# hrz2000/CustomNeRF

Hardware: AMD Instinct MI355X
Metric: training rays/s (higher is better)
Workload: dtype f16

## Files before the change

### customnerf_amd/csrc/grid_fwd_eval.h

```cpp
#pragma once
#include "grid_common.h"

__device__ __forceinline__ float gf_mix_lo(float w, uint32_t g2, float negzero) {
    float r;
    asm("v_fma_mix_f32 %0, %1, %2, %3 op_sel_hi:[0,1,0]" : "=v"(r) : "v"(w), "v"(g2), "v"(negzero));
    return r;
}
__device__ __forceinline__ float gf_mix_hi(float w, uint32_t g2, float negzero) {
    float r;
    asm("v_fma_mix_f32 %0, %1, %2, %3 op_sel:[0,1,0] op_sel_hi:[0,1,0]" : "=v"(r) : "v"(w), "v"(g2), "v"(negzero));
    return r;
}
__device__ __forceinline__ void gf_accum(cn_gf_h2 &acc, float w, uint32_t g2, float negzero) {
    const float p0 = gf_mix_lo(w, g2, negzero), p1 = gf_mix_hi(w, g2, negzero);
    const cn_gf_h2 p = {(_Float16)p0, (_Float16)p1};
    acc = acc + p;
}
__device__ __forceinline__ uint32_t gf_ld1(const unsigned char *__restrict__ base, uint32_t byte_off) { return *reinterpret_cast<const uint32_t *>(base + byte_off); }
struct __attribute__((packed, aligned(4))) gf_u2 { uint32_t x, y; };
struct alignas(16) gf_u4 { uint32_t x, y, z, w; };

__device__ __forceinline__ uint32_t gf_eval_level(const float (&in)[3], const unsigned char *__restrict__ table, uint32_t size, uint32_t resolution,
                                                  float scale, uint32_t gridtype) {
    float fr[3], om[3];
    uint32_t pg[3];
#pragma unroll
    for (int d = 0; d < 3; d++) {
        const float pos = cn_fma(in[d], scale, 0.5f);
        pg[d] = (uint32_t)floorf(pos);
        fr[d] = pos - (float)pg[d];
        om[d] = 1 - fr[d];
    }
    const float a00 = om[0] * om[1], a10 = fr[0] * om[1], a01 = om[0] * fr[1], a11 = fr[0] * fr[1];
    const float w[8] = {a00 * om[2], a10 * om[2], a01 * om[2], a11 * om[2], a00 * fr[2], a10 * fr[2], a01 * fr[2], a11 * fr[2]};
    uint32_t c[8];
    const int mode = ge_level_mode<3>(gridtype, false, size, resolution);
    if (mode == GE_MODE_DENSE) {
        const uint32_t s1 = resolution + 1, s2 = s1 * s1;
        const uint32_t i00 = (pg[0] + pg[1] * s1 + pg[2] * s2) * 4u;
        const gf_u2 r0 = *reinterpret_cast<const gf_u2 *>(table + i00);
        const gf_u2 r1 = *reinterpret_cast<const gf_u2 *>(table + (i00 + s1 * 4u));
        const gf_u2 r2 = *reinterpret_cast<const gf_u2 *>(table + (i00 + s2 * 4u));
        const gf_u2 r3 = *reinterpret_cast<const gf_u2 *>(table + (i00 + (s1 + s2) * 4u));
        c[0] = r0.x; c[1] = r0.y; c[2] = r1.x; c[3] = r1.y; c[4] = r2.x; c[5] = r2.y; c[6] = r3.x; c[7] = r3.y;
    } else if (mode == GE_MODE_HASH2) {
        const uint32_t mask = size - 1;
        const uint32_t hy0 = pg[1] * 2654435761u, hy1 = hy0 + 2654435761u, hz0 = pg[2] * 805459861u, hz1 = hz0 + 805459861u;
        const uint32_t x0 = pg[0], xm = x0 ^ (x0 + 1);
        const bool in_quad = (xm & mask) < 4u;
        const bool odd = (x0 & 1u) != 0;
        const uint32_t hyz[4] = {hy0 ^ hz0, hy1 ^ hz0, hy0 ^ hz1, hy1 ^ hz1};
        uint32_t i0[4];
        gf_u4 v[4];
#pragma unroll
        for (int q = 0; q < 4; q++) {
            i0[q] = (x0 ^ hyz[q]) & mask;
            v[q] = *reinterpret_cast<const gf_u4 *>(table + ((i0[q] & ~3u) * 4u));
        }
        uint32_t far[4] = {0u, 0u, 0u, 0u};
        if (!in_quad) {
#pragma unroll
            for (int q = 0; q < 4; q++) far[q] = gf_ld1(table, ((i0[q] ^ xm) & mask) * 4u);
        }
#pragma unroll
        for (int q = 0; q < 4; q++) {
            const bool b0 = (i0[q] & 1u) != 0, b1 = (i0[q] & 2u) != 0;
            const uint32_t plo = b1 ? v[q].z : v[q].x, phi = b1 ? v[q].w : v[q].y;
            c[2 * q] = b0 ? phi : plo;
            const uint32_t same = b0 ? plo : phi;
            const uint32_t olo = b1 ? v[q].x : v[q].z, ohi = b1 ? v[q].y : v[q].w;
            const uint32_t cross = b0 ? olo : ohi;
            const uint32_t near = odd ? cross : same;
            c[2 * q + 1] = in_quad ? near : far[q];
        }
    } else {
        const uint32_t mask = size - 1, step = resolution + 1;
        const uint32_t s1 = step <= size ? step : 0u;
        const uint32_t s2 = (s1 && step * step <= size) ? step * step : 0u;
        const uint32_t lin = pg[0] + pg[1] * s1 + pg[2] * s2;
        const uint32_t row[4] = {lin, lin + s1, lin + s2, lin + s1 + s2};
        gf_u2 r[4];
        uint32_t i0[4];
#pragma unroll
        for (int q = 0; q < 4; q++) {
            i0[q] = row[q] & mask;
            r[q] = *reinterpret_cast<const gf_u2 *>(table + (i0[q] == mask ? i0[q] - 1 : i0[q]) * 4u);
        }
        bool any_wrap = false;
#pragma unroll
        for (int q = 0; q < 4; q++) any_wrap = any_wrap || i0[q] == mask;
        uint32_t first = 0u;
        if (any_wrap) first = gf_ld1(table, 0u);
#pragma unroll
        for (int q = 0; q < 4; q++) {
            const bool wrap = i0[q] == mask;
            c[2 * q] = wrap ? r[q].y : r[q].x;
            c[2 * q + 1] = wrap ? first : r[q].y;
        }
    }
    const float negzero = -0.0f;
    cn_gf_h2 acc = {(_Float16)0, (_Float16)0};
#pragma unroll
    for (int k = 0; k < 8; k++) gf_accum(acc, w[k], c[k], negzero);
    return __builtin_bit_cast(uint32_t, acc);
}
```

### customnerf_amd/csrc/gridencoder.hip

```cpp
#include "grid_common.h"

template <typename T, int D, int C>
__global__ void __launch_bounds__(GE_BLOCK) k_grid_fwd(const float *__restrict__ inputs, const T *__restrict__ grid, const GridLevels lv,
                                                       T *__restrict__ outputs, uint32_t B, uint32_t L, uint32_t n_levels, uint32_t nb,
                                                       T *__restrict__ dy_dx, uint32_t gridtype, int align_corners, uint32_t interp, int swizzle,
                                                       uint32_t ostride) {
    uint32_t level, pb;
    if (!ge_work_item(nb, n_levels, swizzle, lv, level, pb)) return;
    const uint32_t b = pb * GE_BLOCK + threadIdx.x;
    if (b >= B) return;

    using Vec = FeatVec<T, C>;
    const Vec *__restrict__ table = reinterpret_cast<const Vec *>(grid) + lv.offset[level];
    Vec *out = reinterpret_cast<Vec *>(outputs) + ((size_t)level * ostride + b);

    float in[D];
    bool oob = false;
    ge_load_coords<D>(inputs, b, in);
#pragma unroll
    for (int d = 0; d < D; d++) oob = oob || (in[d] < 0 || in[d] > 1);
    if (oob) {
        Vec z;
#pragma unroll
        for (int c = 0; c < C; c++) z.v[c] = ge_from_float<T>(0.0f);
        *out = z;
        if (dy_dx) {
            T *dd = dy_dx + (size_t)b * D * L * C + (size_t)level * D * C;
#pragma unroll
            for (int i = 0; i < D * C; i++) dd[i] = ge_from_float<T>(0.0f);
        }
        return;
    }

    const uint32_t hashmap_size = lv.size[level];
    const float scale = lv.scale[level];
    const uint32_t resolution = lv.resolution[level];

    float pos[D], pos_deriv[D];
    uint32_t pos_grid[D];
#pragma unroll
    for (int d = 0; d < D; d++) {
        pos[d] = cn_fma(in[d], scale, align_corners ? 0.0f : 0.5f);
        const float fl = floorf(pos[d]);
        pos_grid[d] = (uint32_t)fl;
        pos[d] -= (float)pos_grid[d];
        if (interp == 1) {
            pos_deriv[d] = ge_smoothstep_derivative(pos[d]);
            pos[d] = ge_smoothstep(pos[d]);
        } else {
            pos_deriv[d] = 1.0f;
        }
    }

    struct alignas(sizeof(T) * C) VecPair { Vec a, b; };
    struct alignas(sizeof(T) * C * 4) VecQuad { Vec e[4]; };
    Vec corner[1 << D];
    float wgt[1 << D];
    bool quad = false;
    if constexpr (sizeof(Vec) == 4) {
        quad = gridtype == 0 && ((lv.offset[level] | hashmap_size) & 3u) == 0 && ge_is_hashed<D>(align_corners, hashmap_size, resolution);
    }
    ge_dispatch_mode(ge_level_mode<D>(gridtype, align_corners, hashmap_size, resolution), [&](auto mode_c) {
#pragma unroll
    for (int q = 0; q < (1 << (D - 1)); q++) {
        uint32_t pgl[D];
#pragma unroll
        for (int d = 1; d < D; d++) pgl[d] = (((2 * q) & (1 << d)) == 0) ? pos_grid[d] : pos_grid[d] + 1;
        float w0 = 1 - pos[0], w1 = pos[0];
#pragma unroll
        for (int d = 1; d < D; d++) {
            const float f = (((2 * q) & (1 << d)) == 0) ? (1 - pos[d]) : pos[d];
            w0 *= f; w1 *= f;
        }
        wgt[2 * q] = w0; wgt[2 * q + 1] = w1;
        pgl[0] = pos_grid[0];
        const uint32_t i0 = ge_index_m<D, decltype(mode_c)::value>(gridtype, align_corners, hashmap_size, resolution, pgl);
        pgl[0] = pos_grid[0] + 1;
        const uint32_t i1 = ge_index_m<D, decltype(mode_c)::value>(gridtype, align_corners, hashmap_size, resolution, pgl);
        if (quad) {
            if constexpr (sizeof(Vec) == 4) {
                const VecQuad v = *reinterpret_cast<const VecQuad *>(table + (i0 & ~3u));
                const uint32_t k0 = i0 & 3u, k1 = i1 & 3u;
                const Vec a01 = (k0 & 1) ? v.e[1] : v.e[0], a23 = (k0 & 1) ? v.e[3] : v.e[2];
                corner[2 * q] = (k0 & 2) ? a23 : a01;
                const Vec b01 = (k1 & 1) ? v.e[1] : v.e[0], b23 = (k1 & 1) ? v.e[3] : v.e[2];
                Vec e1 = (k1 & 2) ? b23 : b01;
                if ((i0 ^ i1) > 3u) e1 = table[i1];
                corner[2 * q + 1] = e1;
            }
        } else {
            const uint32_t lo = min(i0, i1), hi_ = max(i0, i1);
            const uint32_t b = (lo + 1 < hashmap_size) ? lo : lo - 1;
            const VecPair v = *reinterpret_cast<const VecPair *>(table + b);
            const Vec e_lo = (b == lo) ? v.a : v.b;
            Vec e_hi = v.b;
            if (hi_ - lo != 1) e_hi = table[hi_];
            corner[2 * q] = (i0 == lo) ? e_lo : e_hi;
            corner[2 * q + 1] = (i0 == lo) ? e_hi : e_lo;
        }
    }
    });
    Vec res;
    if constexpr (sizeof(T) == 2 && C == 2) {
        __half2 r2 = __floats2half2_rn(0.0f, 0.0f);
#pragma unroll
        for (int idx = 0; idx < (1 << D); idx++) ge_accum2(r2, wgt[idx], *reinterpret_cast<const __half2 *>(&corner[idx]));
        res = *reinterpret_cast<const Vec *>(&r2);
    } else {
#pragma unroll
        for (int c = 0; c < C; c++) res.v[c] = ge_from_float<T>(0.0f);
#pragma unroll
        for (int idx = 0; idx < (1 << D); idx++) {
#pragma unroll
            for (int c = 0; c < C; c++) ge_accum(res.v[c], wgt[idx], corner[idx].v[c]);
        }
    }
    *out = res;

    if (dy_dx) {
        T *dd = dy_dx + (size_t)b * D * L * C + (size_t)level * D * C;
#pragma unroll
        for (int gd = 0; gd < D; gd++) {
            T rg[C];
#pragma unroll
            for (int c = 0; c < C; c++) rg[c] = ge_from_float<T>(0.0f);
#pragma unroll
            for (int idx = 0; idx < (1 << (D - 1)); idx++) {
                float w = scale;
                uint32_t pgl[D];
#pragma unroll
                for (int nd = 0; nd < D - 1; nd++) {
                    const int d = (nd >= gd) ? (nd + 1) : nd;
                    if ((idx & (1 << nd)) == 0) { w *= 1 - pos[d]; pgl[d] = pos_grid[d]; }
                    else { w *= pos[d]; pgl[d] = pos_grid[d] + 1; }
                }
                pgl[gd] = pos_grid[gd];
                const Vec left = table[ge_index<D>(gridtype, align_corners, hashmap_size, resolution, pgl)];
                pgl[gd] = pos_grid[gd] + 1;
                const Vec right = table[ge_index<D>(gridtype, align_corners, hashmap_size, resolution, pgl)];
#pragma unroll
                for (int c = 0; c < C; c++) {
                    if constexpr (sizeof(T) == 2) {
                        const float diff = __half2float(__float2half_rn(ge_opaque(__half2float(right.v[c]) - __half2float(left.v[c]))));
                        const float prod = ge_opaque(w * diff * pos_deriv[gd]);
                        rg[c] = __float2half_rn(ge_opaque(__half2float(rg[c]) + __half2float(__float2half_rn(prod))));
                    } else {
                        const float diff = right.v[c] - left.v[c];
                        rg[c] = cn_fma(w * diff, pos_deriv[gd], rg[c]);
                    }
                }
            }
#pragma unroll
            for (int c = 0; c < C; c++) dd[gd * C + c] = rg[c];
        }
    }
}

#include "grid_fwd_eval.h"

__global__ void __launch_bounds__(GE_BLOCK) k_grid_fwd_fast(const float *__restrict__ inputs, const __half *__restrict__ grid, const GridLevels lv,
                                                            __half *__restrict__ outputs, uint32_t B, uint32_t n_levels, uint32_t nb, uint32_t gridtype,
                                                            int swizzle, uint32_t ostride) {
    uint32_t level, pb;
    if (!ge_work_item(nb, n_levels, swizzle, lv, level, pb)) return;
    const uint32_t b = pb * GE_BLOCK + threadIdx.x;
    if (b >= B) return;
    uint32_t *out = reinterpret_cast<uint32_t *>(outputs) + ((size_t)level * ostride + b);
    float in[3];
    ge_load_coords<3>(inputs, b, in);
    if (in[0] < 0 || in[0] > 1 || in[1] < 0 || in[1] > 1 || in[2] < 0 || in[2] > 1) { *out = 0u; return; }

    const unsigned char *__restrict__ table = reinterpret_cast<const unsigned char *>(grid) + (size_t)lv.offset[level] * 4;
    *out = gf_eval_level(in, table, lv.size[level], lv.resolution[level], lv.scale[level], gridtype);
}

template <int SPT>
__global__ void __launch_bounds__(GE_BLOCK) k_grid_fwd_fast_sm(const float *__restrict__ inputs, const __half *__restrict__ grid, const GridLevels lv,
                                                               __half *__restrict__ outputs, uint32_t B, uint32_t n_levels, uint32_t gridtype,
                                                               uint32_t ostride) {
    const uint32_t t0 = blockIdx.x * (GE_BLOCK * SPT) + threadIdx.x;
    if (t0 >= B) return;
    float in[SPT][3];
    bool ok[SPT];
#pragma unroll
    for (int s = 0; s < SPT; s++) {
        ge_load_coords<3>(inputs, min(t0 + s * GE_BLOCK, B - 1), in[s]);
        ok[s] = !(in[s][0] < 0 || in[s][0] > 1 || in[s][1] < 0 || in[s][1] > 1 || in[s][2] < 0 || in[s][2] > 1);
#pragma unroll
        for (int d = 0; d < 3; d++) in[s][d] = ok[s] ? in[s][d] : 0.5f;
    }
    uint32_t *out = reinterpret_cast<uint32_t *>(outputs);
    for (uint32_t i = 0; i < n_levels; i++) {
        const uint32_t level = lv.order[i];
        const unsigned char *__restrict__ table = reinterpret_cast<const unsigned char *>(grid) + (size_t)lv.offset[level] * 4;
        const uint32_t size = lv.size[level], res = lv.resolution[level];
        const float scale = lv.scale[level];
#pragma unroll
        for (int s = 0; s < SPT; s++) {
            const uint32_t b = t0 + s * GE_BLOCK;
            const uint32_t r = gf_eval_level(in[s], table, size, res, scale, gridtype);
            if (b < B) out[(size_t)level * ostride + b] = ok[s] ? r : 0u;
        }
    }
}

template <typename T, int D, int C>
__global__ void __launch_bounds__(GE_BLOCK) k_grid_bwd(const T *__restrict__ grad, const float *__restrict__ inputs, const GridLevels lv,
                                                       float *__restrict__ grad_grid, uint32_t B, uint32_t n_levels, uint32_t nb,
                                                       uint32_t gridtype, int align_corners, uint32_t interp, int swizzle, float *__restrict__ found_inf) {
    uint32_t level, pb;
    if (!ge_work_item(nb, n_levels, swizzle, lv, level, pb)) return;
    const uint32_t b = pb * GE_BLOCK + threadIdx.x;
    if (b >= B) return;

    float in[D];
#pragma unroll
    for (int d = 0; d < D; d++) {
        in[d] = inputs[(size_t)b * D + d];
        if (in[d] < 0 || in[d] > 1) return;
    }
    using Vec = FeatVec<T, C>;
    const Vec g = reinterpret_cast<const Vec *>(grad)[(size_t)level * B + b];
    float *__restrict__ gtable = grad_grid + (size_t)lv.offset[level] * C;
    const uint32_t hashmap_size = lv.size[level];
    const float scale = lv.scale[level];
    const uint32_t resolution = lv.resolution[level];

    float pos[D];
    uint32_t pos_grid[D];
#pragma unroll
    for (int d = 0; d < D; d++) {
        pos[d] = cn_fma(in[d], scale, align_corners ? 0.0f : 0.5f);
        pos_grid[d] = (uint32_t)floorf(pos[d]);
        pos[d] -= (float)pos_grid[d];
        if (interp == 1) pos[d] = ge_smoothstep(pos[d]);
    }
    float gf[C];
#pragma unroll
    for (int c = 0; c < C; c++) {
        gf[c] = ge_to_float(g.v[c]);
        if (!(fabsf(gf[c]) <= 3.4e38f) && found_inf) *found_inf = 1.0f;
    }
#pragma unroll
    for (int idx = 0; idx < (1 << D); idx++) {
        float w = 1;
        uint32_t pgl[D];
#pragma unroll
        for (int d = 0; d < D; d++) {
            if ((idx & (1 << d)) == 0) { w *= 1 - pos[d]; pgl[d] = pos_grid[d]; }
            else { w *= pos[d]; pgl[d] = pos_grid[d] + 1; }
        }
        const uint32_t index = ge_index<D>(gridtype, align_corners, hashmap_size, resolution, pgl) * C;
#pragma unroll
        for (int c = 0; c < C; c++) unsafeAtomicAdd(&gtable[index + c], w * gf[c]);
    }
}

template <typename T, int D, int C>
__global__ void __launch_bounds__(GE_BLOCK) k_input_bwd(const T *__restrict__ grad, const T *__restrict__ dy_dx, float *__restrict__ grad_inputs,
                                                        uint32_t B, uint32_t L) {
    const uint32_t t = threadIdx.x + blockIdx.x * blockDim.x;
    if (t >= B * D) return;
    const uint32_t b = t / D, d = t - b * D;
    const T *dd = dy_dx + (size_t)b * L * D * C;
    float result = 0;
    for (uint32_t l = 0; l < L; l++) {
#pragma unroll
        for (int c = 0; c < C; c++)
            result = cn_fma(ge_to_float(grad[(size_t)l * B * C + (size_t)b * C + c]), ge_to_float(dd[l * D * C + d * C + c]), result);
    }
    grad_inputs[t] = result;
}

template <int D, int C>
__global__ void __launch_bounds__(GE_BLOCK) k_grad_tv(const float *__restrict__ inputs, const float *__restrict__ grid, float *__restrict__ grad,
                                                      const GridLevels lv, float weight, uint32_t B, uint32_t n_levels, uint32_t nb,
                                                      uint32_t gridtype, int align_corners) {
    uint32_t level, pb;
    if (!ge_work_item(nb, n_levels, 0, lv, level, pb)) return;
    const uint32_t b = pb * GE_BLOCK + threadIdx.x;
    if (b >= B) return;
    float in[D];
#pragma unroll
    for (int d = 0; d < D; d++) {
        in[d] = inputs[(size_t)b * D + d];
        if (in[d] < 0 || in[d] > 1) return;
    }
    const float *__restrict__ table = grid + (size_t)lv.offset[level] * C;
    float *__restrict__ gtable = grad + (size_t)lv.offset[level] * C;
    const uint32_t hashmap_size = lv.size[level], resolution = lv.resolution[level];
    const float scale = lv.scale[level];
    uint32_t pos_grid[D];
#pragma unroll
    for (int d = 0; d < D; d++) pos_grid[d] = (uint32_t)floorf(cn_fma(in[d], scale, align_corners ? 0.0f : 0.5f));
    float results[C], idelta[C];
#pragma unroll
    for (int c = 0; c < C; c++) { results[c] = 0; idelta[c] = 0; }
    const uint32_t index = ge_index<D>(gridtype, align_corners, hashmap_size, resolution, pos_grid) * C;
    const float w = weight / (2 * D);
#pragma unroll
    for (int d = 0; d < D; d++) {
        const uint32_t cur_d = pos_grid[d];
        if (cur_d < resolution) {
            pos_grid[d] = cur_d + 1;
            const uint32_t ir = ge_index<D>(gridtype, align_corners, hashmap_size, resolution, pos_grid) * C;
#pragma unroll
            for (int c = 0; c < C; c++) {
                const float gv = table[index + c] - table[ir + c];
                results[c] += gv;
                idelta[c] = cn_fma(gv, gv, idelta[c]);
            }
        }
        if (cur_d > 0) {
            pos_grid[d] = cur_d - 1;
            const uint32_t il = ge_index<D>(gridtype, align_corners, hashmap_size, resolution, pos_grid) * C;
#pragma unroll
            for (int c = 0; c < C; c++) {
                const float gv = table[index + c] - table[il + c];
                results[c] += gv;
                idelta[c] = cn_fma(gv, gv, idelta[c]);
            }
        }
        pos_grid[d] = cur_d;
    }
#pragma unroll
    for (int c = 0; c < C; c++) unsafeAtomicAdd(&gtable[index + c], w * results[c] * (1.0f / sqrtf(idelta[c] + 1e-9f)));
}

__global__ void __launch_bounds__(256) k_cast_f32_f16(const float *__restrict__ src, __half *__restrict__ dst, uint64_t n) {
    const uint64_t n8 = n / 8;
    const uint64_t stride = (uint64_t)gridDim.x * blockDim.x;
    for (uint64_t i = (uint64_t)blockIdx.x * blockDim.x + threadIdx.x; i < n8; i += stride) {
        const float4 a = reinterpret_cast<const float4 *>(src)[i * 2], b = reinterpret_cast<const float4 *>(src)[i * 2 + 1];
        union { __half2 h[4]; uint4 u; } o;
        o.h[0] = __floats2half2_rn(a.x, a.y);
        o.h[1] = __floats2half2_rn(a.z, a.w);
        o.h[2] = __floats2half2_rn(b.x, b.y);
        o.h[3] = __floats2half2_rn(b.z, b.w);
        reinterpret_cast<uint4 *>(dst)[i] = o.u;
    }
    for (uint64_t i = n8 * 8 + (uint64_t)blockIdx.x * blockDim.x + threadIdx.x; i < n; i += stride) dst[i] = __float2half_rn(src[i]);
}

static int ge_swizzle_default() {
    static const int v = cn_tune_env("CNERF_GRID_SWIZZLE", 2);
    return v;
}
static double ge_dense_weight() {
    static const double w = cn_tune_env_f("CNERF_GRID_DENSE_W", 0.7);
    return w;
}

static bool ge_fast_eligible(const GridLevels &lv, uint32_t nl, uint32_t gridtype) {
    static const int on = cn_tune_env("CNERF_GRID_FAST", 1);
    if (!on) return false;
    for (uint32_t l = 0; l < nl; l++) {
        const uint64_t step = (uint64_t)lv.resolution[l] + 1, cells = step * step * step;
        const uint32_t size = lv.size[l];
        const bool pow2 = (size & (size - 1)) == 0;
        if (size >= (1u << 24)) return false;
        if (cells <= size) continue;
        if (!pow2 || size < 8) return false;
        if (gridtype == 0 && ((lv.offset[l] | size) & 3u)) return false;
    }
    return true;
}

#define GE_TRAV_LEVEL 0u
#define GE_TRAV_SAMPLE 1u
#ifndef GE_FAST_SPT
#define GE_FAST_SPT 16
#endif

template <typename T, int D>
static int ge_fwd_C(const float *inputs, const T *emb, const GridLevels &lv, T *out, uint32_t B, uint32_t C, uint32_t L, uint32_t nl, T *dy_dx,
                    uint32_t gridtype, int ac, uint32_t interp, hipStream_t st, uint32_t ostride, uint32_t traversal = GE_TRAV_LEVEL) {
    uint32_t nb = cn_div_up(B, GE_BLOCK);
    const dim3 block(GE_BLOCK);
    int sw = ge_swizzle_default();
    if (sw == 2 && cn_tune_env("CNERF_GRID_SWIZZLE", -1) < 0) {
        uint64_t biggest = 0;
        for (uint32_t l = 0; l < nl; l++) biggest = biggest > lv.size[l] ? biggest : lv.size[l];
        if (biggest * C * sizeof(T) > (4ull << 20)) sw = 0;
    }
    GridLevels lvb = lv;
    if constexpr (std::is_same<T, __half>::value && D == 3) {
        if (C == 2 && !dy_dx && interp == 0 && !ac && ge_fast_eligible(lvb, nl, gridtype)) {
            static const int force = cn_tune_env("CNERF_GRID_TRAV", -1);
            if (force >= 0) traversal = (uint32_t)force;
            if (traversal == GE_TRAV_SAMPLE) {
                static const int spt = cn_tune_env("CNERF_GRID_SPT", GE_FAST_SPT);
#define GE_SM(SPT_) case SPT_: hipLaunchKernelGGL(k_grid_fwd_fast_sm<SPT_>, dim3(cn_div_up(B, GE_BLOCK * SPT_)), block, 0, st, inputs, emb, lvb, out, B, nl, gridtype, ostride); break;
                switch (spt) { GE_SM(4) GE_SM(8) GE_SM(32) default: GE_SM(16) }
#undef GE_SM
                return cn_launch_status();
            }
        }
    }
    dim3 grid(nb * nl);
    if (sw == 2) grid = dim3(CN_NXCD * ge_balance(lvb, nl, nb, D, gridtype, ac != 0, ge_dense_weight()));
    const GridLevels &lv_ = lvb;
    if constexpr (std::is_same<T, __half>::value && D == 3) {
        if (C == 2 && !dy_dx && interp == 0 && !ac && ge_fast_eligible(lv_, nl, gridtype)) {
            hipLaunchKernelGGL(k_grid_fwd_fast, grid, block, 0, st, inputs, emb, lv_, out, B, nl, nb, gridtype, sw, ostride);
            return cn_launch_status();
        }
    }
    switch (C) {
        case 1: hipLaunchKernelGGL((k_grid_fwd<T, D, 1>), grid, block, 0, st, inputs, emb, lv_, out, B, L, nl, nb, dy_dx, gridtype, ac, interp, sw, ostride); break;
        case 2: hipLaunchKernelGGL((k_grid_fwd<T, D, 2>), grid, block, 0, st, inputs, emb, lv_, out, B, L, nl, nb, dy_dx, gridtype, ac, interp, sw, ostride); break;
        case 4: hipLaunchKernelGGL((k_grid_fwd<T, D, 4>), grid, block, 0, st, inputs, emb, lv_, out, B, L, nl, nb, dy_dx, gridtype, ac, interp, sw, ostride); break;
        case 8: hipLaunchKernelGGL((k_grid_fwd<T, D, 8>), grid, block, 0, st, inputs, emb, lv_, out, B, L, nl, nb, dy_dx, gridtype, ac, interp, sw, ostride); break;
        default: return CNERF_EINVAL;
    }
    return cn_launch_status();
}

template <typename T>
static int ge_fwd_D(const float *inputs, const T *emb, const GridLevels &lv, T *out, uint32_t B, uint32_t D, uint32_t C, uint32_t L, uint32_t nl,
                    T *dy_dx, uint32_t gridtype, int ac, uint32_t interp, hipStream_t st, uint32_t ostride, uint32_t traversal = GE_TRAV_LEVEL) {
    switch (D) {
        case 2: return ge_fwd_C<T, 2>(inputs, emb, lv, out, B, C, L, nl, dy_dx, gridtype, ac, interp, st, ostride);
        case 3: return ge_fwd_C<T, 3>(inputs, emb, lv, out, B, C, L, nl, dy_dx, gridtype, ac, interp, st, ostride, traversal);
        case 4: return ge_fwd_C<T, 4>(inputs, emb, lv, out, B, C, L, nl, dy_dx, gridtype, ac, interp, st, ostride);
        case 5: return ge_fwd_C<T, 5>(inputs, emb, lv, out, B, C, L, nl, dy_dx, gridtype, ac, interp, st, ostride);
        default: return CNERF_EINVAL;
    }
}

template <typename T, int D>
static int ge_bwd_C(const T *grad, const float *inputs, const GridLevels &lv, float *gemb, uint32_t B, uint32_t C, uint32_t L, uint32_t nl,
                    const T *dy_dx, float *grad_inputs, uint32_t gridtype, int ac, uint32_t interp, hipStream_t st) {
    const uint32_t nb = cn_div_up(B, GE_BLOCK);
    const dim3 grid(nb * nl), block(GE_BLOCK);
    const int sw = ge_swizzle_default() ? 1 : 0;
    const dim3 gin(cn_div_up(B * D, GE_BLOCK));
    switch (C) {
        case 1:
            hipLaunchKernelGGL((k_grid_bwd<T, D, 1>), grid, block, 0, st, grad, inputs, lv, gemb, B, nl, nb, gridtype, ac, interp, sw, g_cn_found_inf);
            if (dy_dx) hipLaunchKernelGGL((k_input_bwd<T, D, 1>), gin, block, 0, st, grad, dy_dx, grad_inputs, B, L);
            break;
        case 2:
            hipLaunchKernelGGL((k_grid_bwd<T, D, 2>), grid, block, 0, st, grad, inputs, lv, gemb, B, nl, nb, gridtype, ac, interp, sw, g_cn_found_inf);
            if (dy_dx) hipLaunchKernelGGL((k_input_bwd<T, D, 2>), gin, block, 0, st, grad, dy_dx, grad_inputs, B, L);
            break;
        case 4:
            hipLaunchKernelGGL((k_grid_bwd<T, D, 4>), grid, block, 0, st, grad, inputs, lv, gemb, B, nl, nb, gridtype, ac, interp, sw, g_cn_found_inf);
            if (dy_dx) hipLaunchKernelGGL((k_input_bwd<T, D, 4>), gin, block, 0, st, grad, dy_dx, grad_inputs, B, L);
            break;
        case 8:
            hipLaunchKernelGGL((k_grid_bwd<T, D, 8>), grid, block, 0, st, grad, inputs, lv, gemb, B, nl, nb, gridtype, ac, interp, sw, g_cn_found_inf);
            if (dy_dx) hipLaunchKernelGGL((k_input_bwd<T, D, 8>), gin, block, 0, st, grad, dy_dx, grad_inputs, B, L);
            break;
        default: return CNERF_EINVAL;
    }
    return cn_launch_status();
}

template <typename T>
static int ge_bwd_D(const T *grad, const float *inputs, const GridLevels &lv, float *gemb, uint32_t B, uint32_t D, uint32_t C, uint32_t L,
                    uint32_t nl, const T *dy_dx, float *grad_inputs, uint32_t gridtype, int ac, uint32_t interp, hipStream_t st) {
    switch (D) {
        case 2: return ge_bwd_C<T, 2>(grad, inputs, lv, gemb, B, C, L, nl, dy_dx, grad_inputs, gridtype, ac, interp, st);
        case 3: return ge_bwd_C<T, 3>(grad, inputs, lv, gemb, B, C, L, nl, dy_dx, grad_inputs, gridtype, ac, interp, st);
        case 4: return ge_bwd_C<T, 4>(grad, inputs, lv, gemb, B, C, L, nl, dy_dx, grad_inputs, gridtype, ac, interp, st);
        case 5: return ge_bwd_C<T, 5>(grad, inputs, lv, gemb, B, C, L, nl, dy_dx, grad_inputs, gridtype, ac, interp, st);
        default: return CNERF_EINVAL;
    }
}

template <int D>
static int ge_tv_C(const float *inputs, const float *emb, float *grad, const GridLevels &lv, float weight, uint32_t B, uint32_t C, uint32_t L,
                   uint32_t gridtype, int ac, hipStream_t st) {
    const uint32_t nb = cn_div_up(B, GE_BLOCK);
    const dim3 grid(nb * L), block(GE_BLOCK);
    switch (C) {
        case 1: hipLaunchKernelGGL((k_grad_tv<D, 1>), grid, block, 0, st, inputs, emb, grad, lv, weight, B, L, nb, gridtype, ac); break;
        case 2: hipLaunchKernelGGL((k_grad_tv<D, 2>), grid, block, 0, st, inputs, emb, grad, lv, weight, B, L, nb, gridtype, ac); break;
        case 4: hipLaunchKernelGGL((k_grad_tv<D, 4>), grid, block, 0, st, inputs, emb, grad, lv, weight, B, L, nb, gridtype, ac); break;
        case 8: hipLaunchKernelGGL((k_grad_tv<D, 8>), grid, block, 0, st, inputs, emb, grad, lv, weight, B, L, nb, gridtype, ac); break;
        default: return CNERF_EINVAL;
    }
    return cn_launch_status();
}

bool bn_eligible(uint32_t B, uint32_t D, uint32_t C, uint32_t nl, const GridLevels &lv);
uint64_t bn_workspace_bytes(uint32_t B, uint32_t nl, const GridLevels &lv, int dtype);
int bn_backward(const void *grad, const float *inputs, const GridLevels &lv, float *gemb, uint32_t B, uint32_t nl, uint32_t gridtype, int ac,
                uint32_t interp, int dtype, void *workspace, hipStream_t st, bool prepared);
int bn_prepare(const float *inputs, const GridLevels &lv, uint32_t B, uint32_t nl, uint32_t gridtype, int ac, uint32_t interp, int dtype,
               void *workspace, hipStream_t st);
bool bn_needs_plan(uint32_t B, uint32_t nl, const GridLevels &lv, int dtype, uint32_t gridtype);
void bn_grid_adam_arm(const CnerfGridAdam *cfg);
int bn_grid_adam_consumed();
#define BN_MIN_UPDATES (1u << 20)

extern "C" {

int cnerf_grid_backward_adam(const CnerfGridAdam *cfg) {
    if (cfg) {
        if (!cfg->p || !cfg->g || !cfg->m || !cfg->v || !cfg->scaler_state) return CNERF_ENULL;
        if (cfg->n == 0 || (cfg->n & 3) || ((((uintptr_t)cfg->p) | ((uintptr_t)cfg->g) | ((uintptr_t)cfg->m) | ((uintptr_t)cfg->v)) & 15) ||
            (((uintptr_t)cfg->p_half) & 7))
            return CNERF_EINVAL;
        if (!(cfg->beta1 >= 0.0f && cfg->beta1 < 1.0f) || !(cfg->beta2 >= 0.0f && cfg->beta2 < 1.0f) || !(cfg->eps >= 0.0f)) return CNERF_EINVAL;
    }
    bn_grid_adam_arm(cfg);
    return CNERF_OK;
}

int cnerf_grid_backward_adam_consumed(int *yes) {
    if (!yes) return CNERF_ENULL;
    *yes = bn_grid_adam_consumed();
    return CNERF_OK;
}

int cnerf_grid_encode_forward_ordered(const float *inputs, const void *embeddings, const int32_t *offsets_host, void *outputs, uint32_t B, uint32_t D,
                                      uint32_t C, uint32_t L, uint32_t max_level, float S, uint32_t H, void *dy_dx, uint32_t gridtype, int align_corners,
                                      uint32_t interp, int dtype, uint32_t out_level_stride, uint32_t traversal, void *stream) {
    if (gridtype > 1 || interp > 1 || traversal > GE_TRAV_SAMPLE) return CNERF_EINVAL;
    GridLevels lv;
    const uint32_t nl = max_level < L ? max_level : L;
    int rc = ge_levels(offsets_host, L, nl, S, H, lv);
    if (rc) return rc;
    if (D < 2 || D > 5 || !(C == 1 || C == 2 || C == 4 || C == 8)) return CNERF_EINVAL;
    if (dtype != CNERF_F32 && dtype != CNERF_F16) return CNERF_EINVAL;
    if (out_level_stride == 0) out_level_stride = B;
    if (out_level_stride < B) return CNERF_EINVAL;
    if (B == 0 || nl == 0) return CNERF_OK;
    if (!inputs || !embeddings || !outputs) return CNERF_ENULL;
    if (dtype == CNERF_F32)
        return ge_fwd_D<float>(inputs, (const float *)embeddings, lv, (float *)outputs, B, D, C, L, nl, (float *)dy_dx, gridtype, align_corners, interp,
                               CN_STREAM(stream), out_level_stride);
    return ge_fwd_D<__half>(inputs, (const __half *)embeddings, lv, (__half *)outputs, B, D, C, L, nl, (__half *)dy_dx, gridtype, align_corners, interp,
                            CN_STREAM(stream), out_level_stride, traversal);
}

int cnerf_grid_encode_forward_strided(const float *inputs, const void *embeddings, const int32_t *offsets_host, void *outputs, uint32_t B, uint32_t D,
                                      uint32_t C, uint32_t L, uint32_t max_level, float S, uint32_t H, void *dy_dx, uint32_t gridtype, int align_corners,
                                      uint32_t interp, int dtype, uint32_t out_level_stride, void *stream) {
    return cnerf_grid_encode_forward_ordered(inputs, embeddings, offsets_host, outputs, B, D, C, L, max_level, S, H, dy_dx, gridtype, align_corners, interp,
                                             dtype, out_level_stride, GE_TRAV_LEVEL, stream);
}

int cnerf_grid_encode_forward(const float *inputs, const void *embeddings, const int32_t *offsets_host, void *outputs, uint32_t B, uint32_t D,
                              uint32_t C, uint32_t L, uint32_t max_level, float S, uint32_t H, void *dy_dx, uint32_t gridtype, int align_corners,
// ... 123 lines not shown
```

### customnerf_amd/nerf/network_grid.py

```python
import torch
from torch import nn

from .renderer import NeRFRenderer
from .encoding import get_encoder, get_embedder
from .provider_utils import trunc_exp
from .. import tcnn
from ..field import field, field_attach, field_forward_raw, field_forward_rows, packed_weights
from ..gridencoder import GridEncoder


class RGB_network(nn.Module):

    def __init__(self, input_ch_views, opt=None):
        super().__init__()
        self.opt = opt
        cfg = {"otype": "FullyFusedMLP", "activation": "ReLU", "output_activation": "Sigmoid", "n_neurons": 64, "n_hidden_layers": 1}
        self.rgb_network = tcnn.Network(input_ch_views + 64, 3, cfg, seed=13)
        if getattr(opt, 'mask_no_dir', False):
            self.conf_network = tcnn.Network(64, 1, cfg, seed=14)
        else:
            ndim = 1 if getattr(opt, 'keyword2', None) is None else 2
            self.conf_network = tcnn.Network(input_ch_views + 64, ndim, cfg, seed=14)

    def forward(self, x):
        if getattr(self.opt, 'mask_no_dir', False):
            dir_dim = x.shape[-1] - 64
            _, fea = x.split([dir_dim, 64], dim=-1)
            rgb = self.rgb_network(x)
            rgb2 = self.conf_network(fea if getattr(self.opt, 'mask_no_dir_nodetach', False) else fea.detach())
        else:
            rgb = self.rgb_network(x)
            rgb2 = self.conf_network(x.detach())
        return torch.cat([rgb, rgb2], dim=-1)


class NeRFNetwork(NeRFRenderer):
    def __init__(self, opt, device=None, **unused):
        super().__init__(opt)
        grid_type = getattr(opt, 'grid_type', 'tiledgrid')
        self.pos_en, self.pos_en_dim = get_encoder(
            grid_type, input_dim=3,
            num_levels=getattr(opt, 'num_levels', 16), level_dim=getattr(opt, 'level_dim', 2),
            base_resolution=getattr(opt, 'base_resolution', 16),
            log2_hashmap_size=getattr(opt, 'log2_hashmap_size', 21),
            desired_resolution=getattr(opt, 'desired_resolution', 8192))
        n_geo = getattr(opt, 'n_hidden_geo', 2)
        self.network = tcnn.Network(self.pos_en_dim, 64, {"otype": "FullyFusedMLP", "activation": "ReLU", "output_activation": "None",
                                                          "n_neurons": 64, "n_hidden_layers": n_geo}, seed=10)
        self.density_network = tcnn.Network(64, 1, {"otype": "FullyFusedMLP", "activation": "ReLU", "output_activation": "None",
                                                    "n_neurons": 64, "n_hidden_layers": 1}, seed=11)
        self.dir_en, input_ch_views = get_embedder(4)
        sig = {"otype": "FullyFusedMLP", "activation": "ReLU", "output_activation": "Sigmoid", "n_neurons": 64, "n_hidden_layers": 1}
        if getattr(opt, 'train_conf', 0):
            if getattr(opt, 'detach_mask_from_field', False) or getattr(opt, 'mask_no_dir', False):
                self.rgb_network = RGB_network(input_ch_views, opt=opt)
            else:
                self.rgb_network = tcnn.Network(input_ch_views + 64, 3 + 1, sig, seed=12)
        else:
            self.rgb_network = tcnn.Network(input_ch_views + 64, 3, sig, seed=12)
        self.bg_net = None
        self.supports_dir_group = True

    def background(self, d):
        return torch.zeros(d.size(), dtype=d.dtype, device=d.device)

    def gaussian(self, x):
        d = (x ** 2).sum(-1)
        return 5 * torch.exp(-d / (2 * 0.2 ** 2))

    def _fused_cfg(self):
        cfg = getattr(self, '_fused_cfg_cache', None)
        if cfg is None:
            ok = (getattr(self.opt, 'fused_field', True) and isinstance(self.pos_en, GridEncoder) and self.pos_en.level_dim == 2
                  and self.pos_en.input_dim == 3 and self.pos_en.output_dim <= 64 and isinstance(self.rgb_network, tcnn.Network)
                  and self.network.n_hidden_layers in (1, 2) and self.density_network.n_hidden_layers == 1
                  and self.rgb_network.n_hidden_layers == 1 and self.rgb_network.n_output_dims in (3, 4))
            cfg = (self.pos_en.output_dim, self.network.n_hidden_layers, self.rgb_network.n_output_dims) if ok else False
            self._fused_cfg_cache = cfg
        return cfg

    def _half(self):
        return self.network.compute_dtype == torch.float16

    def _weight_image(self):
        if not self.__dict__.get('packed_field_weights') or not self._half():
            return None
        enc_dim, n_geo, n_rgb = self._fused_cfg()
        return packed_weights(self.__dict__.setdefault('_wimg_cache', {}), enc_dim, n_geo, n_rgb, self.network.params, self.density_network.params,
                              self.rgb_network.params)

    def _geo(self, x):
        x_en = self.pos_en(x, bound=self.opt.bound)
        fea = self.network(x_en)
        sigma = self.density_network(fea)
        sigma = trunc_exp(sigma.squeeze(-1) + self.gaussian(x))
        return fea, sigma

    def forward(self, x, d, l=None, ratio=1, shading='albedo', dir_group=1):
        cfg = self._fused_cfg()
        if cfg and x.is_cuda:
            enc_dim, n_geo, n_rgb = cfg
            x = x.reshape(-1, 3)
            enc = self.pos_en.encode(x, bound=self.opt.bound, half=self._half())
            sigma, rgbc = field(enc, x, d.reshape(-1, 3), dir_group, enc_dim, n_geo, n_rgb, self.network.params, self.density_network.params,
                                self.rgb_network.params, wimg=self._weight_image())
            return sigma, (rgbc if n_rgb == 4 else rgbc[:, :3]), None
        if dir_group != 1:
            d = d.reshape(-1, 3).repeat_interleave(dir_group, dim=0)[:x.reshape(-1, 3).shape[0]]
        fea, sigma = self._geo(x)
        view_en = self.dir_en(d)
        rgb_input = torch.cat([view_en.to(fea.dtype), fea], dim=-1)
        radiances = self.rgb_network(rgb_input)
        return sigma, radiances, None

    def density(self, x):
        cfg = self._fused_cfg()
        if cfg and x.is_cuda and not torch.is_grad_enabled():
            enc_dim, n_geo, n_rgb = cfg
            x = x.reshape(-1, 3).contiguous().float()
            enc = self.pos_en.encode(x, bound=self.opt.bound, half=self._half())
            sigma, _ = field_forward_raw(enc, x, None, 1, enc_dim, n_geo, n_rgb, self.network.params, self.density_network.params, None,
                                         with_rgb=False, wimg=self._weight_image())
            return {'sigma': sigma}
        return {'sigma': self._geo(x)[1]}

    @property
    def supports_split_eval(self):
        return bool(self._fused_cfg())

    def split_buffers(self, P, device):
        dt = torch.float16 if self._half() else torch.float32
        L = self.pos_en.num_levels
        return torch.empty(L, P, 2, dtype=dt, device=device), torch.empty(P, 3, dtype=torch.float32, device=device)

    @torch.no_grad()
    def split_encode(self, enc, unit, x, row0, unit_ready=False, importance=False):
        B = x.shape[0]
        u = unit[row0:row0 + B]
        if not unit_ready:
            torch.add(x, self.opt.bound, out=u)
            u.div_(2 * self.opt.bound)
        trav = 0
        if importance and getattr(self.opt, 'tune_gather_traversal', True):
            trav = self.__dict__.get('_fine_tuner')
            if trav is None:
                from ..gridencoder.grid import TraversalTuner
                trav = self.__dict__['_fine_tuner'] = TraversalTuner()
        self.pos_en.encode_into(u, enc, row0, half=self._half(), traversal=trav)

    @torch.no_grad()
    def split_density(self, enc, x):
        enc_dim, n_geo, n_rgb = self._fused_cfg()
        sigma, _ = field_forward_raw(enc, x, None, 1, enc_dim, n_geo, n_rgb, self.network.params, self.density_network.params, None, with_rgb=False,
                                     wimg=self._weight_image())
        return sigma

    def _overlap_plan(self):
        return getattr(self.opt, 'overlap_scatter_plan', True)

    def split_prepare(self, unit, grad_enabled):
        if not (grad_enabled and self.pos_en.embeddings.requires_grad and self._overlap_plan()):
            return None
        if not getattr(self.opt, 'early_scatter_plan', True):
            return None
        return self.pos_en.prepare_backward(unit, self._half())

    def split_forward(self, enc, unit, x, d, dir_group, plan=None):
        enc_dim, n_geo, n_rgb = self._fused_cfg()
        if torch.is_grad_enabled() and self.pos_en.embeddings.requires_grad:
            enc = self.pos_en.attach_backward(enc, unit, overlap=self._overlap_plan(), plan=plan)
        sigma, rgbc = field(enc, x, d.reshape(-1, 3), dir_group, enc_dim, n_geo, n_rgb, self.network.params, self.density_network.params,
                            self.rgb_network.params, grad_in_place=bool(getattr(self, 'grad_in_place', False)), wimg=self._weight_image())
        return sigma, rgbc

    def split_outputs(self, P, device):
        return torch.empty(P, dtype=torch.float32, device=device), torch.empty(P, 4, dtype=torch.float32, device=device)

    @torch.no_grad()
    def split_forward_rows(self, enc, row0, x_rows, d, dir_group, sigma_all, rgbc_all):
        enc_dim, n_geo, n_rgb = self._fused_cfg()
        n = x_rows.shape[0]
        field_forward_rows(enc, row0, x_rows, d.reshape(-1, 3).contiguous().float(), dir_group, enc_dim, n_geo, n_rgb, self.network.params,
                           self.density_network.params, self.rgb_network.params, sigma_all[row0:row0 + n], rgbc_all[row0:row0 + n],
                           wimg=self._weight_image())

    def split_attach(self, enc, unit, x, d, dir_group, sigma_all, rgbc_all, plan=None):
        if not torch.is_grad_enabled():
            return sigma_all, rgbc_all
        enc_dim, n_geo, n_rgb = self._fused_cfg()
        if self.pos_en.embeddings.requires_grad:
            enc = self.pos_en.attach_backward(enc, unit, overlap=self._overlap_plan(), plan=plan)
        return field_attach(enc, x, d.reshape(-1, 3), dir_group, enc_dim, n_geo, n_rgb, self.network.params, self.density_network.params,
                            self.rgb_network.params, sigma_all, rgbc_all, grad_in_place=bool(getattr(self, 'grad_in_place', False)),
                            wimg=self._weight_image())

    def get_params(self, lr):
        return [
            {'params': self.pos_en.parameters(), 'lr': lr * 10},
            {'params': self.network.parameters(), 'lr': lr},
            {'params': self.density_network.parameters(), 'lr': lr},
            {'params': self.rgb_network.parameters(), 'lr': lr},
        ]
```

### scratch/nan_hunt.py

```python
import json, subprocess, sys, os
n = int(sys.argv[1]) if len(sys.argv) > 1 else 3
for i in range(n):
    out = subprocess.run([sys.executable, "bench.py", "--task", "edit", "--steps", "6", "--warmup", "3", "--no-cpu-baseline", "--no-variants", "--no-roofline"],
                         capture_output=True, text=True)
    try:
        d = json.loads([l for l in out.stdout.splitlines() if l.startswith("{")][-1])
        print(i, os.environ.get("CNERF_GRID_SPT"), os.environ.get("CNERF_GRID_TRAV"), "ms", round(d["ms_per_step"], 2), "loss", d["config"]["final_loss"], "skipped", d["config"]["steps_skipped_on_overflow"], d["config"]["loss_scale"][-12:], flush=True)
    except Exception as e:
        print(i, "FAILED", e, out.stderr[-500:], flush=True)
```

Before: 8.357 million.

## Software-pipeline grid gathers across sample groups and levels in per-sample kernel

Splits grid level evaluation into an issue phase (index math plus table loads into a pending struct) and a combine phase (select corners and interpolate). The per-sample forward kernel double-buffers groups of samples, so the loads for the next group, or the first group of the next level, are issued before the current group is combined, hiding gather latency. The kernel gains templated group size and block size with a waves_per_eu hint, plus a variant table chosen through an env var. Coarse sampling now also gets its own traversal tuner. The cost is higher register pressure and possibly lower occupancy.

Result: faster. 8.449 million, median of 6 (+1.1%).

```diff
diff --git a/customnerf_amd/csrc/grid_fwd_eval.h b/customnerf_amd/csrc/grid_fwd_eval.h
--- a/customnerf_amd/csrc/grid_fwd_eval.h
+++ b/customnerf_amd/csrc/grid_fwd_eval.h
@@ -20,82 +20,115 @@
 struct __attribute__((packed, aligned(4))) gf_u2 { uint32_t x, y; };
 struct alignas(16) gf_u4 { uint32_t x, y, z, w; };
 
-__device__ __forceinline__ uint32_t gf_eval_level(const float (&in)[3], const unsigned char *__restrict__ table, uint32_t size, uint32_t resolution,
-                                                  float scale, uint32_t gridtype) {
-    float fr[3], om[3];
+struct GfPending {
+    gf_u4 v[4];
+    uint32_t far[4];
+    float fr[3];
+    uint32_t sel;
+};
+
+template <int MODE>
+__device__ __forceinline__ void gf_issue(const float (&in)[3], const unsigned char *__restrict__ table, uint32_t size, uint32_t resolution,
+                                         float scale, GfPending &p) {
     uint32_t pg[3];
 #pragma unroll
     for (int d = 0; d < 3; d++) {
         const float pos = cn_fma(in[d], scale, 0.5f);
         pg[d] = (uint32_t)floorf(pos);
-        fr[d] = pos - (float)pg[d];
-        om[d] = 1 - fr[d];
+        p.fr[d] = pos - (float)pg[d];
     }
-    const float a00 = om[0] * om[1], a10 = fr[0] * om[1], a01 = om[0] * fr[1], a11 = fr[0] * fr[1];
-    const float w[8] = {a00 * om[2], a10 * om[2], a01 * om[2], a11 * om[2], a00 * fr[2], a10 * fr[2], a01 * fr[2], a11 * fr[2]};
-    uint32_t c[8];
-    const int mode = ge_level_mode<3>(gridtype, false, size, resolution);
-    if (mode == GE_MODE_DENSE) {
+    if constexpr (MODE == GE_MODE_DENSE) {
         const uint32_t s1 = resolution + 1, s2 = s1 * s1;
         const uint32_t i00 = (pg[0] + pg[1] * s1 + pg[2] * s2) * 4u;
-        const gf_u2 r0 = *reinterpret_cast<const gf_u2 *>(table + i00);
-        const gf_u2 r1 = *reinterpret_cast<const gf_u2 *>(table + (i00 + s1 * 4u));
-        const gf_u2 r2 = *reinterpret_cast<const gf_u2 *>(table + (i00 + s2 * 4u));
-        const gf_u2 r3 = *reinterpret_cast<const gf_u2 *>(table + (i00 + (s1 + s2) * 4u));
-        c[0] = r0.x; c[1] = r0.y; c[2] = r1.x; c[3] = r1.y; c[4] = r2.x; c[5] = r2.y; c[6] = r3.x; c[7] = r3.y;
-    } else if (mode == GE_MODE_HASH2) {
+        const uint32_t off[4] = {i00, i00 + s1 * 4u, i00 + s2 * 4u, i00 + (s1 + s2) * 4u};
+#pragma unroll
+        for (int q = 0; q < 4; q++) {
+            const gf_u2 r = *reinterpret_cast<const gf_u2 *>(table + off[q]);
+            p.v[q] = {r.x, r.y, 0u, 0u};
+            p.far[q] = 0u;
+        }
+        p.sel = 0u;
+    } else if constexpr (MODE == GE_MODE_HASH2) {
         const uint32_t mask = size - 1;
         const uint32_t hy0 = pg[1] * 2654435761u, hy1 = hy0 + 2654435761u, hz0 = pg[2] * 805459861u, hz1 = hz0 + 805459861u;
         const uint32_t x0 = pg[0], xm = x0 ^ (x0 + 1);
         const bool in_quad = (xm & mask) < 4u;
-        const bool odd = (x0 & 1u) != 0;
         const uint32_t hyz[4] = {hy0 ^ hz0, hy1 ^ hz0, hy0 ^ hz1, hy1 ^ hz1};
         uint32_t i0[4];
-        gf_u4 v[4];
 #pragma unroll
         for (int q = 0; q < 4; q++) {
             i0[q] = (x0 ^ hyz[q]) & mask;
-            v[q] = *reinterpret_cast<const gf_u4 *>(table + ((i0[q] & ~3u) * 4u));
+            const gf_u4 t = *reinterpret_cast<const gf_u4 *>(table + ((i0[q] & ~3u) * 4u));
+            p.v[q].x = t.x; p.v[q].y = t.y; p.v[q].z = t.z; p.v[q].w = t.w;
         }
-        uint32_t far[4] = {0u, 0u, 0u, 0u};
+#pragma unroll
+        for (int q = 0; q < 4; q++) p.far[q] = 0u;
         if (!in_quad) {
 #pragma unroll
-            for (int q = 0; q < 4; q++) far[q] = gf_ld1(table, ((i0[q] ^ xm) & mask) * 4u);
+            for (int q = 0; q < 4; q++) p.far[q] = gf_ld1(table, ((i0[q] ^ xm) & mask) * 4u);
         }
-#pragma unroll
-        for (int q = 0; q < 4; q++) {
-            const bool b0 = (i0[q] & 1u) != 0, b1 = (i0[q] & 2u) != 0;
-            const uint32_t plo = b1 ? v[q].z : v[q].x, phi = b1 ? v[q].w : v[q].y;
-            c[2 * q] = b0 ? phi : plo;
-            const uint32_t same = b0 ? plo : phi;
-            const uint32_t olo = b1 ? v[q].x : v[q].z, ohi = b1 ? v[q].y : v[q].w;
-            const uint32_t cross = b0 ? olo : ohi;
-            const uint32_t near = odd ? cross : same;
-            c[2 * q + 1] = in_quad ? near : far[q];
-        }
+        p.sel = (i0[0] & 3u) | ((i0[1] & 3u) << 2) | ((i0[2] & 3u) << 4) | ((i0[3] & 3u) << 6) | ((x0 & 1u) << 8) | (in_quad ? 0u : 512u);
     } else {
+        static_assert(MODE == GE_MODE_TILED2, "gf_issue: DENSE, HASH2 or TILED2");
         const uint32_t mask = size - 1, step = resolution + 1;
         const uint32_t s1 = step <= size ? step : 0u;
         const uint32_t s2 = (s1 && step * step <= size) ? step * step : 0u;
         const uint32_t lin = pg[0] + pg[1] * s1 + pg[2] * s2;
         const uint32_t row[4] = {lin, lin + s1, lin + s2, lin + s1 + s2};
-        gf_u2 r[4];
-        uint32_t i0[4];
+        uint32_t wraps = 0u;
 #pragma unroll
         for (int q = 0; q < 4; q++) {
-            i0[q] = row[q] & mask;
-            r[q] = *reinterpret_cast<const gf_u2 *>(table + (i0[q] == mask ? i0[q] - 1 : i0[q]) * 4u);
+            const uint32_t i0 = row[q] & mask;
+            const gf_u2 r = *reinterpret_cast<const gf_u2 *>(table + (i0 == mask ? i0 - 1 : i0) * 4u);
+            p.v[q] = {r.x, r.y, 0u, 0u};
+            wraps |= (i0 == mask ? 1u : 0u) << q;
         }
-        bool any_wrap = false;
 #pragma unroll
-        for (int q = 0; q < 4; q++) any_wrap = any_wrap || i0[q] == mask;
-        uint32_t first = 0u;
-        if (any_wrap) first = gf_ld1(table, 0u);
+        for (int q = 0; q < 4; q++) p.far[q] = 0u;
+        if (wraps) p.far[0] = gf_ld1(table, 0u);
+        p.sel = wraps;
+    }
+}
+
+template <int MODE>
+__device__ __forceinline__ uint32_t gf_combine(const GfPending &p) {
+    float om[3];
+#pragma unroll
+    for (int d = 0; d < 3; d++) om[d] = 1 - p.fr[d];
+    const float(&fr)[3] = p.fr;
+    const float a00 = om[0] * om[1], a10 = fr[0] * om[1], a01 = om[0] * fr[1], a11 = fr[0] * fr[1];
+    const float w[8] = {a00 * om[2], a10 * om[2], a01 * om[2], a11 * om[2], a00 * fr[2], a10 * fr[2], a01 * fr[2], a11 * fr[2]};
+    uint32_t c[8];
+    if constexpr (MODE == GE_MODE_DENSE) {
 #pragma unroll
         for (int q = 0; q < 4; q++) {
-            const bool wrap = i0[q] == mask;
-            c[2 * q] = wrap ? r[q].y : r[q].x;
-            c[2 * q + 1] = wrap ? first : r[q].y;
+            c[2 * q] = p.v[q].x;
+            c[2 * q + 1] = p.v[q].y;
+        }
+    } else if constexpr (MODE == GE_MODE_HASH2) {
+        const bool odd = (p.sel & 256u) != 0;
+        const bool in_quad = (p.sel & 512u) == 0;
+#pragma unroll
+        for (int q = 0; q < 4; q++) {
+            const bool b0 = (p.sel & (1u << (2 * q))) != 0, b1 = (p.sel & (2u << (2 * q))) != 0;
+            const uint32_t vx = p.v[q].x, vy = p.v[q].y, vz = p.v[q].z, vw = p.v[q].w;
+            const uint32_t plo = b1 ? vz : vx, phi = b1 ? vw : vy;
+            c[2 * q] = b0 ? phi : plo;
+            const uint32_t same = b0 ? plo : phi;
+            const uint32_t olo = b1 ? vx : vz, ohi = b1 ? vy : vw;
+            const uint32_t cross = b0 ? olo : ohi;
+            const uint32_t near = odd ? cross : same;
+            const uint32_t far = p.far[q];
+            c[2 * q + 1] = in_quad ? near : far;
+        }
+    } else {
+        static_assert(MODE == GE_MODE_TILED2, "gf_combine: DENSE, HASH2 or TILED2");
+#pragma unroll
+        for (int q = 0; q < 4; q++) {
+            const bool wrap = (p.sel & (1u << q)) != 0;
+            const uint32_t vx = p.v[q].x, vy = p.v[q].y, first = p.far[0];
+            c[2 * q] = wrap ? vy : vx;
+            c[2 * q + 1] = wrap ? first : vy;
         }
     }
     const float negzero = -0.0f;
@@ -104,3 +137,22 @@
     for (int k = 0; k < 8; k++) gf_accum(acc, w[k], c[k], negzero);
     return __builtin_bit_cast(uint32_t, acc);
 }
+
+template <typename F>
+__device__ __forceinline__ void gf_dispatch_mode(int mode, F &&f) {
+    if (mode == GE_MODE_DENSE) f(std::integral_constant<int, GE_MODE_DENSE>{});
+    else if (mode == GE_MODE_HASH2) f(std::integral_constant<int, GE_MODE_HASH2>{});
+    else f(std::integral_constant<int, GE_MODE_TILED2>{});
+}
+
+__device__ __forceinline__ uint32_t gf_eval_level(const float (&in)[3], const unsigned char *__restrict__ table, uint32_t size, uint32_t resolution,
+                                                  float scale, uint32_t gridtype) {
+    const int mode = ge_level_mode<3>(gridtype, false, size, resolution);
+    uint32_t r = 0u;
+    gf_dispatch_mode(mode, [&](auto m) {
+        GfPending p;
+        gf_issue<decltype(m)::value>(in, table, size, resolution, scale, p);
+        r = gf_combine<decltype(m)::value>(p);
+    });
+    return r;
+}
diff --git a/customnerf_amd/csrc/gridencoder.hip b/customnerf_amd/csrc/gridencoder.hip
--- a/customnerf_amd/csrc/gridencoder.hip
+++ b/customnerf_amd/csrc/gridencoder.hip
@@ -174,33 +174,87 @@
     *out = gf_eval_level(in, table, lv.size[level], lv.resolution[level], lv.scale[level], gridtype);
 }
 
-template <int SPT>
-__global__ void __launch_bounds__(GE_BLOCK) k_grid_fwd_fast_sm(const float *__restrict__ inputs, const __half *__restrict__ grid, const GridLevels lv,
-                                                               __half *__restrict__ outputs, uint32_t B, uint32_t n_levels, uint32_t gridtype,
-                                                               uint32_t ostride) {
-    const uint32_t t0 = blockIdx.x * (GE_BLOCK * SPT) + threadIdx.x;
+struct GfSmLevel {
+    const unsigned char *table;
+    uint32_t level, size, res;
+    float scale;
+    int mode;
+};
+__device__ __forceinline__ GfSmLevel gf_sm_level(const __half *grid, const GridLevels &lv, uint32_t i, uint32_t gridtype) {
+    GfSmLevel L;
+    L.level = lv.order[i];
+    L.table = reinterpret_cast<const unsigned char *>(grid) + (size_t)lv.offset[L.level] * 4;
+    L.size = lv.size[L.level];
+    L.res = lv.resolution[L.level];
+    L.scale = lv.scale[L.level];
+    L.mode = ge_level_mode<3>(gridtype, false, L.size, L.res);
+    return L;
+}
+template <int G, int SPT>
+__device__ __forceinline__ void gf_sm_issue(const GfSmLevel &L, const float (&in)[SPT][3], int s0, GfPending (&p)[G]) {
+    gf_dispatch_mode(L.mode, [&](auto m) {
+#pragma unroll
+        for (int k = 0; k < G; k++) gf_issue<decltype(m)::value>(in[s0 + k], L.table, L.size, L.res, L.scale, p[k]);
+    });
+}
+template <int G, int NT>
+__device__ __forceinline__ void gf_sm_combine(const GfSmLevel &L, const GfPending (&p)[G], int s0, uint32_t okbits, uint32_t t0, uint32_t B,
+                                              uint32_t ostride, uint32_t *__restrict__ out) {
+    uint32_t r[G];
+    gf_dispatch_mode(L.mode, [&](auto m) {
+#pragma unroll
+        for (int k = 0; k < G; k++) r[k] = gf_combine<decltype(m)::value>(p[k]);
+    });
+#pragma unroll
+    for (int k = 0; k < G; k++) {
+        const uint32_t b = t0 + (s0 + k) * NT;
+        if (b < B) out[(size_t)L.level * ostride + b] = (okbits >> (s0 + k)) & 1u ? r[k] : 0u;
+    }
+}
+
+template <int SPT, int G, int NT>
+__global__ void __launch_bounds__(NT) __attribute__((amdgpu_waves_per_eu(1))) k_grid_fwd_fast_sm(const float *__restrict__ inputs,
+        const __half *__restrict__ grid, const GridLevels lv, __half *__restrict__ outputs, uint32_t B, uint32_t n_levels, uint32_t gridtype,
+        uint32_t ostride) {
+    static_assert(SPT % (2 * G) == 0 && SPT <= 32, "an even number of groups per level (the two buffers alternate by group)");
+    constexpr int NG = SPT / G;
+    const uint32_t t0 = blockIdx.x * (NT * SPT) + threadIdx.x;
     if (t0 >= B) return;
+    GeCoords<3> raw[SPT];
+#pragma unroll
+    for (int s = 0; s < SPT; s++) raw[s] = reinterpret_cast<const GeCoords<3> *>(inputs)[min(t0 + s * NT, B - 1)];
     float in[SPT][3];
-    bool ok[SPT];
+    uint32_t okbits = 0u;
 #pragma unroll
     for (int s = 0; s < SPT; s++) {
-        ge_load_coords<3>(inputs, min(t0 + s * GE_BLOCK, B - 1), in[s]);
-        ok[s] = !(in[s][0] < 0 || in[s][0] > 1 || in[s][1] < 0 || in[s][1] > 1 || in[s][2] < 0 || in[s][2] > 1);
-#pragma unroll
-        for (int d = 0; d < 3; d++) in[s][d] = ok[s] ? in[s][d] : 0.5f;
+        const float *c = raw[s].v;
+        const bool ok = !(c[0] < 0 || c[0] > 1 || c[1] < 0 || c[1] > 1 || c[2] < 0 || c[2] > 1);
+        okbits |= (ok ? 1u : 0u) << s;
+#pragma unroll
+        for (int d = 0; d < 3; d++) in[s][d] = ok ? c[d] : 0.5f;
     }
     uint32_t *out = reinterpret_cast<uint32_t *>(outputs);
-    for (uint32_t i = 0; i < n_levels; i++) {
-        const uint32_t level = lv.order[i];
-        const unsigned char *__restrict__ table = reinterpret_cast<const unsigned char *>(grid) + (size_t)lv.offset[level] * 4;
-        const uint32_t size = lv.size[level], res = lv.resolution[level];
-        const float scale = lv.scale[level];
-#pragma unroll
-        for (int s = 0; s < SPT; s++) {
-            const uint32_t b = t0 + s * GE_BLOCK;
-            const uint32_t r = gf_eval_level(in[s], table, size, res, scale, gridtype);
-            if (b < B) out[(size_t)level * ostride + b] = ok[s] ? r : 0u;
-        }
+    GfPending pa[G], pb[G];
+    GfSmLevel cur = gf_sm_level(grid, lv, 0, gridtype);
+    gf_sm_issue<G>(cur, in, 0, pa);
+    for (uint32_t i = 0; i + 1 < n_levels; i++) {
+        const GfSmLevel nxt = gf_sm_level(grid, lv, i + 1, gridtype);
+#pragma unroll
+        for (int g = 0; g < NG; g += 2) {
+            gf_sm_issue<G>(cur, in, (g + 1) * G, pb);
+            gf_sm_combine<G, NT>(cur, pa, g * G, okbits, t0, B, ostride, out);
+            if (g + 2 < NG) gf_sm_issue<G>(cur, in, (g + 2) * G, pa);
+            else gf_sm_issue<G>(nxt, in, 0, pa);
+            gf_sm_combine<G, NT>(cur, pb, (g + 1) * G, okbits, t0, B, ostride, out);
+        }
+        cur = nxt;
+    }
+#pragma unroll
+    for (int g = 0; g < NG; g += 2) {
+        gf_sm_issue<G>(cur, in, (g + 1) * G, pb);
+        gf_sm_combine<G, NT>(cur, pa, g * G, okbits, t0, B, ostride, out);
+        if (g + 2 < NG) gf_sm_issue<G>(cur, in, (g + 2) * G, pa);
+        gf_sm_combine<G, NT>(cur, pb, (g + 1) * G, okbits, t0, B, ostride, out);
     }
 }
 
@@ -368,9 +422,7 @@
 
 #define GE_TRAV_LEVEL 0u
 #define GE_TRAV_SAMPLE 1u
-#ifndef GE_FAST_SPT
-#define GE_FAST_SPT 16
-#endif
+#define GE_SM_VARIANTS(X) X(0, 16, 4, 256) X(1, 16, 2, 256) X(2, 8, 4, 256) X(3, 8, 2, 256) X(4, 8, 2, 512)
 
 template <typename T, int D>
 static int ge_fwd_C(const float *inputs, const T *emb, const GridLevels &lv, T *out, uint32_t B, uint32_t C, uint32_t L, uint32_t nl, T *dy_dx,
@@ -389,9 +441,9 @@
             static const int force = cn_tune_env("CNERF_GRID_TRAV", -1);
             if (force >= 0) traversal = (uint32_t)force;
             if (traversal == GE_TRAV_SAMPLE) {
-                static const int spt = cn_tune_env("CNERF_GRID_SPT", GE_FAST_SPT);
-#define GE_SM(SPT_) case SPT_: hipLaunchKernelGGL(k_grid_fwd_fast_sm<SPT_>, dim3(cn_div_up(B, GE_BLOCK * SPT_)), block, 0, st, inputs, emb, lvb, out, B, nl, gridtype, ostride); break;
-                switch (spt) { GE_SM(4) GE_SM(8) GE_SM(32) default: GE_SM(16) }
+                static const int variant = cn_tune_env("CNERF_GRID_SM", 0);
+#define GE_SM(V_, SPT_, G_, NT_) case V_: hipLaunchKernelGGL((k_grid_fwd_fast_sm<SPT_, G_, NT_>), dim3(cn_div_up(B, SPT_ * NT_)), dim3(NT_), 0, st, inputs, emb, lvb, out, B, nl, gridtype, ostride); break;
+                switch (variant) { GE_SM_VARIANTS(GE_SM) default: return CNERF_EINVAL; }
 #undef GE_SM
                 return cn_launch_status();
             }
diff --git a/customnerf_amd/nerf/network_grid.py b/customnerf_amd/nerf/network_grid.py
--- a/customnerf_amd/nerf/network_grid.py
+++ b/customnerf_amd/nerf/network_grid.py
@@ -141,11 +141,12 @@
             torch.add(x, self.opt.bound, out=u)
             u.div_(2 * self.opt.bound)
         trav = 0
-        if importance and getattr(self.opt, 'tune_gather_traversal', True):
-            trav = self.__dict__.get('_fine_tuner')
+        if getattr(self.opt, 'tune_gather_traversal', True):
+            key = '_fine_tuner' if importance else '_coarse_tuner'
+            trav = self.__dict__.get(key)
             if trav is None:
                 from ..gridencoder.grid import TraversalTuner
-                trav = self.__dict__['_fine_tuner'] = TraversalTuner()
+                trav = self.__dict__[key] = TraversalTuner()
         self.pos_en.encode_into(u, enc, row0, half=self._half(), traversal=trav)
 
     @torch.no_grad()
diff --git a/scratch/nan_hunt.py b/scratch/nan_hunt.py
--- a/scratch/nan_hunt.py
+++ b/scratch/nan_hunt.py
@@ -5,6 +5,6 @@
                          capture_output=True, text=True)
     try:
         d = json.loads([l for l in out.stdout.splitlines() if l.startswith("{")][-1])
-        print(i, os.environ.get("CNERF_GRID_SPT"), os.environ.get("CNERF_GRID_TRAV"), "ms", round(d["ms_per_step"], 2), "loss", d["config"]["final_loss"], "skipped", d["config"]["steps_skipped_on_overflow"], d["config"]["loss_scale"][-12:], flush=True)
+        print(i, os.environ.get("CNERF_GRID_SM"), os.environ.get("CNERF_GRID_TRAV"), "ms", round(d["ms_per_step"], 2), "loss", d["config"]["final_loss"], "skipped", d["config"]["steps_skipped_on_overflow"], d["config"]["loss_scale"][-12:], flush=True)
     except Exception as e:
         print(i, "FAILED", e, out.stderr[-500:], flush=True)
```
